# skypilot-org/skypilot

Hardware: AMD Instinct MI355X
Metric: tokens/sec (node) sky-launched Llama-3-8B (higher is better)
Workload: dtype bf16; 1 GPU; model=llama3-8b, global_batch=6, seq_len=4096, parallelism=dp1, sky_launched=True

## Files before the change

### skypilot_amd/models/llama.py

```python
from __future__ import annotations

import math
from dataclasses import dataclass

import torch
import torch.nn as nn

from skypilot_amd import ops


@dataclass
class LlamaConfig:
    name: str = "llama3-8b"
    vocab_size: int = 128256
    hidden_size: int = 4096
    intermediate_size: int = 14336
    num_layers: int = 32
    num_heads: int = 32
    num_kv_heads: int = 8
    head_dim: int = 128
    rope_theta: float = 500000.0
    norm_eps: float = 1e-5
    max_seq_len: int = 8192
    tie_embeddings: bool = False
# ... 100 lines not shown
        k = lin(x, self.wk.weight, self.wk.bias).view(B, S, self.n_kv, d)
        v = lin(x, self.wv.weight, self.wv.bias).view(B, S, self.n_kv, d)
        q = ops.rope(q.reshape(B * S, self.n_q, d), cos, sin,
                     positions).view(B, S, self.n_q, d)
        k = ops.rope(k.reshape(B * S, self.n_kv, d), cos, sin,
                     positions).view(B, S, self.n_kv, d)
        if infer_ctx is None:
            o = ops.attention(q, k, v, self.scale, causal=True)
        elif infer_ctx.mode == "append":
            o = append_attention(self, q, k, v, infer_ctx)
        else:
            slots = (infer_ctx.prefill_slots
                     if infer_ctx.prefill_slots is not None
                     else [infer_ctx.prefill_slot])
            lens = (infer_ctx.prefill_lens
                    if infer_ctx.prefill_lens is not None
                    else [infer_ctx.prefill_len])
            for i, (slot, ln) in enumerate(zip(slots, lens)):
                infer_ctx.cache.write_prefill(self.layer_idx, slot,
                                              k[i:i + 1], v[i:i + 1], ln)
            o = ops.attention(q, k, v, self.scale, causal=True)
        return lin(o.reshape(B, S, self.n_q * d), self.wo.weight)


class MLP(nn.Module):
    def __init__(self, cfg: LlamaConfig):
        super().__init__()
        h, m = cfg.hidden_size, cfg.intermediate_size
        self.w_gate_up = nn.Linear(h, 2 * m, bias=False)
        self.w_down = nn.Linear(m, h, bias=False)
        self.m = m

    def forward(self, x, infer_ctx=None):
        decode = infer_ctx is not None and infer_ctx.mode == "decode"
        lin = ops.decode_linear if decode else torch.nn.functional.linear
        return lin(ops.swiglu(lin(x, self.w_gate_up.weight)),
                   self.w_down.weight)

    def down_from_gu(self, gu):
        return ops.decode_linear(ops.swiglu(gu), self.w_down.weight)



class Block(nn.Module):
    def __init__(self, cfg: LlamaConfig, layer_idx: int):
        super().__init__()
        self.attn = Attention(cfg)
        self.attn.layer_idx = layer_idx
        self.mlp = MLP(cfg)
        self.attn_norm = nn.Parameter(torch.ones(cfg.hidden_size))
        self.mlp_norm = nn.Parameter(torch.ones(cfg.hidden_size))
        self.eps = cfg.norm_eps

    def forward(self, x, cos, sin, positions, infer_ctx=None):
        x = x + self.attn(ops.rmsnorm(x, self.attn_norm, self.eps), cos, sin,
                          positions, infer_ctx)
        x = x + self.mlp(ops.rmsnorm(x, self.mlp_norm, self.eps),
                         infer_ctx)
        return x


class Llama(nn.Module):
    def __init__(self, cfg: LlamaConfig):
        super().__init__()
        self.cfg = cfg
        self.embed = nn.Embedding(cfg.vocab_size, cfg.hidden_size)
        self.blocks = nn.ModuleList(
            Block(cfg, i) for i in range(cfg.num_layers))
        self.final_norm = nn.Parameter(torch.ones(cfg.hidden_size))
        self.lm_head = nn.Linear(cfg.hidden_size, cfg.vocab_size, bias=False)
        if cfg.tie_embeddings:
            self.lm_head.weight = self.embed.weight
        self._rope = None

    def _tables(self, device):
        if self._rope is None or self._rope[0].device != device:
            self._rope = rope_tables(self.cfg, device)
        return self._rope

    def forward(self, tokens: torch.Tensor, positions: torch.Tensor = None,
                infer_ctx=None) -> torch.Tensor:
        B, S = tokens.shape
        cos, sin = self._tables(tokens.device)
        if positions is None:
            positions = torch.arange(S, dtype=torch.int32,
                                     device=tokens.device)
            positions = positions.unsqueeze(0).expand(B, S).reshape(-1)
        x = self.embed(tokens)
        if infer_ctx is not None and infer_ctx.mode == "decode":
            res = None
            for blk in self.blocks:
                if not hasattr(blk.attn, "_wqkv"):
                    if res is None:
                        h = ops.rmsnorm(x, blk.attn_norm, blk.eps)
                    else:
                        x, h = ops.rmsnorm_res(x, res, blk.attn_norm,
                                               blk.eps)
                    a = blk.attn(h, cos, sin, positions, infer_ctx)
                    x, h2 = ops.rmsnorm_res(x, a, blk.mlp_norm, blk.eps)
                    res = blk.mlp(h2, infer_ctx)
                    continue
                x, qkv = ops.decode_norm_linear(
                    x, res, blk.attn_norm, blk.eps, blk.attn.packed_qkv())
                a = blk.attn(None, cos, sin, positions, infer_ctx,
                             qkv=qkv)
                x, gu = ops.decode_norm_linear(
                    x, a, blk.mlp_norm, blk.eps, blk.mlp.w_gate_up.weight)
                res = blk.mlp.down_from_gu(gu)
            _, logits = ops.decode_norm_linear(
                x, res, self.final_norm, self.cfg.norm_eps,
                self.lm_head.weight)
            return logits
        for blk in self.blocks:
            x = blk(x, cos, sin, positions, infer_ctx)
        if infer_ctx is not None and infer_ctx.mode == "append":
            last = (infer_ctx.append_lens.long() - 1).clamp(min=0)
            x = x[torch.arange(B, device=x.device), last].unsqueeze(1)
        x = ops.rmsnorm(x, self.final_norm, self.cfg.norm_eps)
        return self.lm_head(x)

    def loss(self, tokens: torch.Tensor, targets: torch.Tensor):
        logits = self.forward(tokens)
        return ops.fused_cross_entropy(
            logits.reshape(-1, self.cfg.vocab_size), targets.reshape(-1))

    def num_params(self) -> int:
        return sum(p.numel() for p in self.parameters())

    def flops_per_token(self, seq_len: int) -> float:
        c = self.cfg
        return 6 * self.num_params() + \
            6 * c.num_layers * 2 * seq_len * c.num_heads * c.head_dim


def build_model(name: str, device="cpu", dtype=torch.bfloat16,
                seed: int = 0) -> Llama:
    cfg = CONFIGS[name]
    torch.manual_seed(seed)
    with torch.device("meta" if device != "cpu" else "cpu"):
        model = Llama(cfg)
    if device != "cpu":
        model = model.to_empty(device=device)
        with torch.no_grad():
            for p in model.parameters():
                p.normal_(0.0, 0.02)
    return model.to(dtype)
```

### skypilot_amd/ops/__init__.py

```python
from __future__ import annotations

import importlib.util
import math
import os
from pathlib import Path

import torch

_C = None
_LOAD_ERR: Exception | None = None


def _load():
    global _C, _LOAD_ERR
    if _C is not None:
        return _C
    so = Path(__file__).resolve().parent / "_C.so"
    try:
        if not so.exists():
            raise ImportError(
                f"native extension {so} not built; run "
                "`python -m skypilot_amd.ops.build`")
        spec = importlib.util.spec_from_file_location("skypilot_amd.ops._C",
                                                      so)
# ... 57 lines not shown
    att = torch.matmul(qf, kf.transpose(-1, -2)) * scale
    if causal:
        mask = torch.triu(torch.ones(S, S, dtype=torch.bool,
                                     device=q.device), 1)
        att = att.masked_fill(mask, float("-inf"))
    p = att.softmax(-1)
    out = torch.matmul(p, vf)
    return out.permute(0, 2, 1, 3).to(q.dtype)


def cross_entropy_ref(logits: torch.Tensor, targets: torch.Tensor,
                      ignore_index: int = -100) -> torch.Tensor:
    return torch.nn.functional.cross_entropy(
        logits.float(), targets.long(), ignore_index=ignore_index,
        reduction="mean")


class _RMSNormFn(torch.autograd.Function):
    @staticmethod
    def forward(ctx, x, w, eps):
        if x.is_cuda:
            C = _require_native("rmsnorm")
            inv_rms = torch.empty(x.numel() // x.shape[-1],
                                  device=x.device, dtype=torch.float32)
            y = C.rmsnorm_fwd(x.contiguous(), w.contiguous(), inv_rms, eps)
            ctx.save_for_backward(x, w, inv_rms)
            ctx.native = True
            return y
        ctx.save_for_backward(x, w)
        ctx.eps = eps
        ctx.native = False
        return rmsnorm_ref(x, w, eps)

    @staticmethod
    def backward(ctx, dy):
        if ctx.native:
            x, w, inv_rms = ctx.saved_tensors
            C = native()
            dx, dw = C.rmsnorm_bwd(x.contiguous(), w.contiguous(),
                                   dy.contiguous(), inv_rms)
            return dx, dw.to(w.dtype), None
        x, w = ctx.saved_tensors
        xf, wf, dyf = x.float(), w.float(), dy.float()
        H = x.shape[-1]
        inv = torch.rsqrt(xf.pow(2).mean(-1, keepdim=True) + ctx.eps)
        dot = (dyf * wf * xf).sum(-1, keepdim=True)
        dx = inv * (dyf * wf - xf * inv * inv * dot / H)
        dw = (dyf * xf * inv).reshape(-1, H).sum(0)
        return dx.to(x.dtype), dw.to(w.dtype), None


def rmsnorm(x: torch.Tensor, w: torch.Tensor, eps: float = 1e-5):
    return _RMSNormFn.apply(x, w, eps)


class _RoPEFn(torch.autograd.Function):
    @staticmethod
    def forward(ctx, x, cos, sin, positions):
        ctx.save_for_backward(cos, sin, positions)
        if x.is_cuda:
            C = _require_native("rope")
            return C.rope(x.contiguous(), cos, sin, positions, False)
        return rope_ref(x, cos, sin, positions)

    @staticmethod
    def backward(ctx, dy):
        cos, sin, positions = ctx.saved_tensors
        if dy.is_cuda:
            C = native()
            return C.rope(dy.contiguous(), cos, sin, positions,
                          True), None, None, None
        return rope_ref(dy, cos, sin, positions, backward=True), \
            None, None, None


def rope(x, cos, sin, positions):
    if x.is_cuda and x.dim() > 3:
        positions = positions.expand(x.shape[:-2]).reshape(-1)
    return _RoPEFn.apply(x, cos, sin, positions)


class _AttentionFn(torch.autograd.Function):
    @staticmethod
    def forward(ctx, q, k, v, scale, causal):
        ctx.scale, ctx.causal = scale, causal
        if q.is_cuda:
            C = _require_native("attention")
            q, k, v = q.contiguous(), k.contiguous(), v.contiguous()
            O, lse = C.attn_fwd(q, k, v, scale, causal)
            ctx.save_for_backward(q, k, v, O, lse)
            ctx.native = True
            return O
        ctx.save_for_backward(q, k, v)
        ctx.native = False
        return attention_ref(q, k, v, scale, causal)

    @staticmethod
    def backward(ctx, dO):
        if ctx.native:
            q, k, v, O, lse = ctx.saved_tensors
            C = native()
            dq, dk, dv = C.attn_bwd(q, k, v, O, dO.contiguous(), lse,
                                    ctx.scale, ctx.causal)
            return dq, dk, dv, None, None
        q, k, v = ctx.saved_tensors
        with torch.enable_grad():
# ... 354 lines not shown

def sample_tokens(logits, temperature, top_p, top_k, seed, counter):
    if not logits.is_cuda:
        return sample_tokens_reference(logits, temperature, top_p, top_k,
                                       seed, counter)
    C = _require_native("sample_tokens")
    if logits.dtype != torch.bfloat16 or logits.dim() != 2:
        raise ValueError("sample_tokens: logits must be bf16 [n, V] on GPU")
    n = logits.shape[0]
    blk = pack_samp(n, temperature, top_p, top_k, seed,
                    counter).to(logits.device)
    toks, tau = C.sample_tokens(logits.contiguous(), blk[:5], blk[5])
    return toks, tau


def decode_sample_advance(logits, stage, ring, ctr, samp):
    C = _require_native("decode_sample_advance")
    C.decode_sample_advance(logits.contiguous(), stage, ring, ctr, samp)


def decode_swiglu_down(gu, weight):
    return decode_linear(swiglu(gu), weight)


def attn_decode_qkv(qkv, kc, vc, cos, sin, positions, kv_lens, slot_ids,
                    Hq, Hkv, scale):
    D = kc.shape[3]
    if qkv.is_cuda and qkv.dtype == torch.bfloat16 and D == 128:
        C = _require_native("attn_decode_qkv")
        return C.attn_decode_qkv(qkv.contiguous(), kc, vc, cos, sin,
                                 positions.int(), kv_lens.int(),
                                 slot_ids.int(), Hq, Hkv, scale)
    q = rope_kvwrite(qkv, kc, vc, cos, sin, positions, slot_ids, Hq, Hkv)
    return attn_decode(q, kc, vc, kv_lens, slot_ids, scale)


def rope_kvwrite(qkv, kc, vc, cos, sin, positions, slot_ids, Hq, Hkv):
    D = kc.shape[3]
    n = qkv.shape[0]
    if qkv.is_cuda and qkv.dtype == torch.bfloat16 and D == 128:
        C = _require_native("rope_kvwrite")
        return C.rope_kvwrite(qkv.contiguous(), kc, vc, cos, sin,
                              positions.int(), slot_ids.int(), Hq, Hkv)
    q, k, v = qkv.split([Hq * D, Hkv * D, Hkv * D], dim=-1)
    qr = rope(q.reshape(n, Hq, D), cos, sin, positions)
    kr = rope(k.reshape(n, Hkv, D), cos, sin, positions)
    pos = positions.long()
    kc[slot_ids.long(), pos] = kr
    vc[slot_ids.long(), pos] = v.reshape(n, Hkv, D)
    return qr


__all__ = [
    "rmsnorm", "rope", "attention", "fused_cross_entropy", "attn_decode",
    "swiglu", "decode_linear", "rmsnorm_res", "rope_kvwrite",
    "decode_swiglu_down",
    "native", "native_available", "rmsnorm_ref", "rope_ref",
    "attention_ref", "cross_entropy_ref", "attn_decode_ref",
    "attn_append", "attn_append_ref",
]
```

### skypilot_amd/ops/csrc/bindings.cpp

```cpp
#include <torch/extension.h>

#include <ATen/hip/HIPContext.h>
#include <hip/hip_runtime.h>

#include <limits>
#include <vector>

#include "attn_append.h"
#include "attn_launch.h"

#define CHECK_GPU(x) TORCH_CHECK(x.is_cuda(), #x " must be on GPU")
#define CHECK_CONTIG(x) TORCH_CHECK(x.is_contiguous(), #x " must be contiguous")
#define CHECK_BF16(x) \
  TORCH_CHECK(x.scalar_type() == at::kBFloat16, #x " must be bf16")

static hipStream_t cur_stream() {
  return at::hip::getCurrentHIPStream().stream();
}

extern "C" {
void rmsnorm_fwd_launch(const void*, const void*, void*, float*, long long,
                        int, float, hipStream_t);
void rmsnorm_bwd_launch(const void*, const void*, const void*, const float*,
                        void*, float*, long long, int, hipStream_t);
void rope_launch(const void*, void*, const float*, const float*, const int*,
                 long long, int, int, bool, hipStream_t);
void adamw_launch(void*, float*, const void*, float*, float*, long long,
                  float, float, float, float, float, int, float, hipStream_t);
void cross_entropy_launch(void*, const int*, float*, long long, int, float,
                          int, hipStream_t);
void mfma_probe_launch(const void*, const void*, float*, hipStream_t);
void mfma32_probe_launch(const void*, const void*, float*, hipStream_t);
void trb16_probe_launch(float*, int, hipStream_t);
void permlane_probe_launch(float*, hipStream_t);
void skinny_gemm_launch(const void*, const void*, void*, int, int, int,
                        hipStream_t);
void skinny_gemm_swiglu_launch(const void*, const void*, void*, int, int,
                               int, hipStream_t);
void transpose_bf16_launch(const void*, void*, int, int, hipStream_t);
void skinny_gemm_fp8_launch(const void*, const float*, const void*, void*,
                            int, int, int, hipStream_t);
void gemm_nt_launch(const void*, const void*, void*, int, int, long long,
                    hipStream_t);
void adamw_mt_launch(const void*, const void*, const void*, const void*,
                     const void*, long long, float, float, float, float,
                     int, float, hipStream_t);
void decode_advance_launch(const void*, long long, void*, long long,
                           void*, const void*, int, hipStream_t);
void sample_tokens_launch(const void*, int, long long, const void*,
                          const void*, void*, void*, hipStream_t);
void decode_sample_advance_launch(const void*, int, void*, long long, void*,
                                  const void*, int, const void*,
                                  hipStream_t);
void rmsnorm_res_launch(const void*, const void*, const void*, void*, void*,
                        int, int, float, hipStream_t);
void rope_kvwrite_launch(const void*, void*, void*, void*, const void*,
                         const void*, const void*, const void*, int, int,
                         int, int, int, hipStream_t);
void swiglu_fwd_launch(const void*, void*, long long, int, hipStream_t);
void swiglu_bwd_launch(const void*, const void*, void*, long long, int,
                       hipStream_t);
void skinny_gemm_fp8_norm_launch(const void*, const float*, const void*,
                                 const void*, const void*, void*, float,
                                 void*, int, int, int, hipStream_t);
void attn_decode_qkv_launch(const void*, void*, void*, void*, const void*,
                            const void*, const int*, const int*,
                            const int*, int, int, int, int, float,
                            hipStream_t);
void attn_decode_launch(const void*, const void*, const void*, void*,
                        const int*, const int*, int, int, int, int, float,
                        hipStream_t);
}

torch::Tensor rmsnorm_fwd(torch::Tensor x, torch::Tensor w,
                          torch::Tensor inv_rms, double eps) {
  CHECK_GPU(x); CHECK_CONTIG(x); CHECK_BF16(x);
  CHECK_GPU(w); CHECK_CONTIG(w); CHECK_BF16(w);
  const int H = (int)x.size(-1);
  TORCH_CHECK(H % 8 == 0, "hidden dim must be a multiple of 8");
  TORCH_CHECK(w.numel() == H, "rmsnorm_fwd: w must have H = ", H,
              " elements, got ", w.numel());
  long long rows = x.numel() / H;
  CHECK_GPU(inv_rms); CHECK_CONTIG(inv_rms);
  TORCH_CHECK(inv_rms.scalar_type() == at::kFloat && inv_rms.numel() == rows,
              "rmsnorm_fwd: inv_rms must be fp32 with one entry per row");
  auto y = torch::empty_like(x);
  rmsnorm_fwd_launch(x.data_ptr(), w.data_ptr(), y.data_ptr(),
                     inv_rms.data_ptr<float>(), rows, H, (float)eps,
                     cur_stream());
  return y;
}

std::vector<torch::Tensor> rmsnorm_bwd(torch::Tensor x, torch::Tensor w,
                                       torch::Tensor dy,
                                       torch::Tensor inv_rms) {
  CHECK_GPU(x); CHECK_CONTIG(x); CHECK_BF16(x);
  CHECK_GPU(w); CHECK_CONTIG(w); CHECK_BF16(w);
  CHECK_GPU(dy); CHECK_CONTIG(dy); CHECK_BF16(dy);
  CHECK_GPU(inv_rms); CHECK_CONTIG(inv_rms);
  const int H = (int)x.size(-1);
  TORCH_CHECK(H % 8 == 0 && H <= 16384,
              "rmsnorm_bwd: hidden dim must be a multiple of 8 and at most "
              "16384, got ", H);
  TORCH_CHECK(w.numel() == H, "rmsnorm_bwd: w must have H = ", H,
              " elements, got ", w.numel());
  TORCH_CHECK(dy.sizes() == x.sizes(), "rmsnorm_bwd: dy must have x's shape");
  long long rows = x.numel() / H;
  TORCH_CHECK(inv_rms.scalar_type() == at::kFloat && inv_rms.numel() == rows,
              "rmsnorm_bwd: inv_rms must be fp32 with one entry per row");
  auto dx = torch::empty_like(x);
  auto dw = torch::zeros({(long)H},
                         x.options().dtype(at::kFloat));
  rmsnorm_bwd_launch(x.data_ptr(), w.data_ptr(), dy.data_ptr(),
                     inv_rms.data_ptr<float>(), dx.data_ptr(),
                     dw.data_ptr<float>(), rows, H, cur_stream());
  return {dx, dw};
}

torch::Tensor rope(torch::Tensor x, torch::Tensor cos_tab,
                   torch::Tensor sin_tab, torch::Tensor positions,
                   bool backward) {
  CHECK_GPU(x); CHECK_CONTIG(x); CHECK_BF16(x);
  TORCH_CHECK(positions.scalar_type() == at::kInt,
              "rope: positions must be int32");
  CHECK_GPU(positions); CHECK_CONTIG(positions);
  TORCH_CHECK(x.dim() >= 2, "rope: x must be [..., heads, head_dim]");
  const int D = (int)x.size(-1);
  const int H = (int)x.size(-2);
  TORCH_CHECK(D % 2 == 0, "rope: head dim must be even, got ", D);
  long long n_tokens = x.numel() / ((long long)H * D);
  TORCH_CHECK(positions.numel() == n_tokens, "rope: need one position per "
              "token: ", n_tokens, " tokens, ", positions.numel(),
              " positions");
  for (const torch::Tensor& t : {cos_tab, sin_tab}) {
    CHECK_GPU(t); CHECK_CONTIG(t);
    TORCH_CHECK(t.scalar_type() == at::kFloat, "rope: cos/sin must be fp32");
    TORCH_CHECK(t.dim() >= 1 && t.size(-1) == D / 2,
                "rope: cos/sin last dim must be head_dim/2 = ", D / 2);
  }
  auto y = torch::empty_like(x);
  rope_launch(x.data_ptr(), y.data_ptr(), cos_tab.data_ptr<float>(),
              sin_tab.data_ptr<float>(), positions.data_ptr<int>(), n_tokens,
              H, D, backward, cur_stream());
  return y;
}

void adamw_step(std::vector<torch::Tensor> params_bf16,
                std::vector<torch::Tensor> params_master,
                std::vector<torch::Tensor> grads,
                std::vector<torch::Tensor> exp_avg,
                std::vector<torch::Tensor> exp_avg_sq, double lr, double beta1,
                double beta2, double eps, double weight_decay, int64_t step,
                double grad_scale, std::vector<bool> decay_mask) {
  auto stream = cur_stream();
  for (size_t i = 0; i < params_bf16.size(); ++i) {
    auto& p = params_bf16[i];
    long long n = p.numel();
    float wd = decay_mask.empty() || decay_mask[i] ? (float)weight_decay : 0.f;
    adamw_launch(p.data_ptr(), params_master[i].data_ptr<float>(),
                 grads[i].data_ptr(), exp_avg[i].data_ptr<float>(),
                 exp_avg_sq[i].data_ptr<float>(), n, (float)lr, (float)beta1,
                 (float)beta2, (float)eps, wd, (int)step, (float)grad_scale,
                 stream);
  }
}

torch::Tensor cross_entropy_fused(torch::Tensor logits, torch::Tensor targets,
                                  double grad_scale, int64_t ignore_index) {
  CHECK_GPU(logits); CHECK_CONTIG(logits); CHECK_BF16(logits);
// ... 397 lines not shown
  const int64_t N = X.size(0), I = X.size(1);
  TORCH_CHECK(N >= 1 && N <= 8, op, ": N must be 1..8, got ", N);
  TORCH_CHECK(I >= 16 && I % 16 == 0 &&
                  I <= std::numeric_limits<int>::max(),
              op, ": I must be a positive multiple of 16, got ", I);
  check_fp8_weight(op, W8, scale, I, X);
  const int64_t O = W8.size(0);
  auto y = torch::empty({N, O}, X.options());
  skinny_gemm_fp8_launch(W8.data_ptr(), scale.data_ptr<float>(),
                         X.data_ptr(), y.data_ptr(), (int)N, (int)I, (int)O,
                         cur_stream());
  return y;
}

torch::Tensor skinny_gemm(torch::Tensor X, torch::Tensor W) {
  CHECK_GPU(X); CHECK_CONTIG(X); CHECK_BF16(X);
  CHECK_GPU(W); CHECK_CONTIG(W); CHECK_BF16(W);
  const int N = (int)X.size(0), I = (int)X.size(1), O = (int)W.size(0);
  TORCH_CHECK(W.size(1) == I, "skinny_gemm: inner dims mismatch");
  TORCH_CHECK(N >= 1 && N <= 8, "skinny_gemm: N must be 1..8");
  TORCH_CHECK(I % 512 == 0, "skinny_gemm: I must be a multiple of 512");
  auto y = torch::empty({N, O}, X.options());
  skinny_gemm_launch(W.data_ptr(), X.data_ptr(), y.data_ptr(), N, I, O,
                     cur_stream());
  return y;
}

std::vector<torch::Tensor> rmsnorm_res(torch::Tensor x, torch::Tensor res,
                                       torch::Tensor w, double eps) {
  const char* op = "rmsnorm_res";
  check_dense(op, "x", x, at::kBFloat16, x);
  TORCH_CHECK(x.dim() >= 1, op, ": x must be [..., H], got a scalar");
  const int64_t H = x.size(-1);
  TORCH_CHECK(H >= 256 && H % 256 == 0 && H <= 8192, op,
              ": H must be a multiple of 256 and <= 8192, got ", H);
  check_dense(op, "res", res, at::kBFloat16, x);
  TORCH_CHECK(res.sizes() == x.sizes(), op, ": res must have x's shape ",
              x.sizes(), ", got ", res.sizes());
  check_dense(op, "w", w, at::kBFloat16, x);
  TORCH_CHECK(w.numel() == H, op, ": w must have H = ", H,
              " elements, got ", w.numel());
  const int64_t rows = x.numel() / H;
  TORCH_CHECK(rows <= std::numeric_limits<int>::max(), op, ": ", rows,
              " rows exceed the grid limit 2^31 - 1");
  auto x_out = torch::empty_like(x);
  auto h_out = torch::empty_like(x);
  if (rows > 0)
    rmsnorm_res_launch(x.data_ptr(), res.data_ptr(), w.data_ptr(),
                       x_out.data_ptr(), h_out.data_ptr(), (int)rows, (int)H,
                       (float)eps, cur_stream());
  return {x_out, h_out};
}

void decode_advance(torch::Tensor logits, torch::Tensor stage,
                    torch::Tensor ring, torch::Tensor ctr) {
  const char* op = "decode_advance";
  check_dense(op, "logits", logits, at::kBFloat16, logits);
  TORCH_CHECK(logits.dim() >= 1, op,
              ": logits must be [b, V], got a scalar");
  const int64_t V = logits.size(-1);
  TORCH_CHECK(V >= 1 && V <= std::numeric_limits<int>::max(), op,
              ": V must be in [1, 2^31 - 1], got ", V);
  const int64_t b = logits.numel() / V;
  check_dense(op, "stage", stage, at::kInt, logits);
  TORCH_CHECK(stage.dim() == 2 && stage.size(0) == 6 && stage.size(1) == b,
              op, ": stage must be [6, b] = [6, ", b, "], got ",
              stage.sizes());
  check_dense(op, "ring", ring, at::kLong, logits);
  TORCH_CHECK(ring.dim() == 2 && ring.size(0) >= 1 &&
                  ring.size(0) <= std::numeric_limits<int>::max() &&
                  ring.size(1) == b,
              op, ": ring must be [chunk >= 1, b] = [chunk, ", b, "], got ",
              ring.sizes());
  check_dense(op, "ctr", ctr, at::kLong, logits);
  TORCH_CHECK(ctr.numel() == 1, op, ": ctr must hold one element, got ",
              ctr.sizes());
  TORCH_CHECK(b <= std::numeric_limits<int>::max(), op, ": b = ", b,
              " rows exceed the grid limit 2^31 - 1");
  if (b > 0)
    decode_advance_launch(logits.data_ptr(), V, stage.data_ptr(), b,
                          ring.data_ptr(), ctr.data_ptr(),
                          (int)ring.size(0), cur_stream());
}

static const long long kSampleMaxV = 1ll << 23;

std::vector<torch::Tensor> sample_tokens(torch::Tensor logits,
                                         torch::Tensor samp,
                                         torch::Tensor counter) {
  CHECK_GPU(logits); CHECK_CONTIG(logits); CHECK_BF16(logits);
  CHECK_GPU(samp); CHECK_CONTIG(samp);
  CHECK_GPU(counter); CHECK_CONTIG(counter);
  TORCH_CHECK(logits.dim() == 2, "sample_tokens: logits must be [n, V]");
  TORCH_CHECK(samp.dtype() == torch::kInt32, "sample_tokens: samp int32");
  TORCH_CHECK(counter.dtype() == torch::kInt32,
              "sample_tokens: counter int32");
  const long long n = logits.size(0);
  const long long V = logits.size(1);
  TORCH_CHECK(V >= 1 && V <= kSampleMaxV,
              "sample_tokens: V must be in [1, 2^23], got ", V);
  TORCH_CHECK(samp.dim() == 2 && samp.size(0) == 5 && samp.size(1) == n,
              "sample_tokens: samp must be [5, n]");
  TORCH_CHECK(counter.dim() == 1 && counter.size(0) == n,
              "sample_tokens: counter must be [n]");
  auto tokens = torch::empty({n}, logits.options().dtype(torch::kInt64));
  auto tau = torch::empty({n}, logits.options().dtype(torch::kFloat));
// ... 79 lines not shown

torch::Tensor swiglu_bwd(torch::Tensor gu, torch::Tensor dy) {
  CHECK_GPU(gu); CHECK_CONTIG(gu); CHECK_BF16(gu);
  CHECK_GPU(dy); CHECK_CONTIG(dy); CHECK_BF16(dy);
  const int M2 = (int)gu.size(-1);
  TORCH_CHECK(M2 % 16 == 0, "swiglu_bwd: last dim must be 2*M with "
              "M % 8 == 0, got ", M2);
  auto ysizes = gu.sizes().vec();
  ysizes.back() = M2 / 2;
  TORCH_CHECK(dy.sizes() == at::IntArrayRef(ysizes),
              "swiglu_bwd: dy must have the shape of swiglu_fwd(gu)");
  long long rows = gu.numel() / M2;
  auto dgu = torch::empty_like(gu);
  swiglu_bwd_launch(gu.data_ptr(), dy.data_ptr(), dgu.data_ptr(), rows,
                    M2 / 2, cur_stream());
  return dgu;
}

torch::Tensor mfma_probe(torch::Tensor A, torch::Tensor B) {
  CHECK_GPU(A); CHECK_BF16(A); CHECK_CONTIG(A); CHECK_CONTIG(B);
  TORCH_CHECK(A.size(0) == 16 && A.size(1) == 32);
  TORCH_CHECK(B.size(0) == 32 && B.size(1) == 16);
  auto C = torch::zeros({16, 16}, A.options().dtype(at::kFloat));
  mfma_probe_launch(A.data_ptr(), B.data_ptr(), C.data_ptr<float>(),
                    cur_stream());
  return C;
}

torch::Tensor mfma32_probe(torch::Tensor A, torch::Tensor B) {
  CHECK_GPU(A); CHECK_BF16(A); CHECK_CONTIG(A); CHECK_CONTIG(B);
  TORCH_CHECK(A.size(0) == 32 && A.size(1) == 16);
  TORCH_CHECK(B.size(0) == 16 && B.size(1) == 32);
  auto C = torch::zeros({32, 32}, A.options().dtype(at::kFloat));
  mfma32_probe_launch(A.data_ptr(), B.data_ptr(), C.data_ptr<float>(),
                      cur_stream());
  return C;
}

torch::Tensor trb16_probe(int64_t mode, torch::Tensor ref_dev) {
  auto out = torch::zeros({64, 4}, ref_dev.options().dtype(at::kFloat));
  trb16_probe_launch(out.data_ptr<float>(), (int)mode, cur_stream());
  return out;
}

torch::Tensor permlane_probe(torch::Tensor ref_dev) {
  auto out = torch::zeros({64, 2}, ref_dev.options().dtype(at::kFloat));
  permlane_probe_launch(out.data_ptr<float>(), cur_stream());
  return out;
}

PYBIND11_MODULE(TORCH_EXTENSION_NAME, m) {
  m.def("rmsnorm_fwd", &rmsnorm_fwd);
  m.def("rmsnorm_bwd", &rmsnorm_bwd);
  m.def("rope", &rope);
  m.def("adamw_step", &adamw_step);
  m.def("cross_entropy_fused", &cross_entropy_fused);
  m.def("attn_fwd", &attn_fwd);
  m.def("attn_bwd", &attn_bwd, py::arg("Q"), py::arg("K"), py::arg("V"),
        py::arg("O"), py::arg("dO"), py::arg("lse"), py::arg("scale"),
        py::arg("causal"), py::arg("dkv_variant") = -1,
        py::arg("dq_variant") = -1);
  m.def("attn_decode", &attn_decode);
  m.def("attn_append", &attn_append);
  m.def("skinny_gemm", &skinny_gemm);
  m.def("skinny_gemm_fp8", &skinny_gemm_fp8);
  m.def("transpose_bf16", &transpose_bf16);
  m.def("gemm_nt", &gemm_nt);
  m.def("wgrad_tn", &wgrad_tn);
  m.def("adamw_step_mt", &adamw_step_mt);
  m.def("skinny_gemm_swiglu", &skinny_gemm_swiglu);
  m.def("rmsnorm_res", &rmsnorm_res);
  m.def("rope_kvwrite", &rope_kvwrite);
  m.def("decode_advance", &decode_advance);
  m.def("sample_tokens", &sample_tokens);
  m.def("decode_sample_advance", &decode_sample_advance);
  m.def("attn_decode_qkv", &attn_decode_qkv);
  m.def("skinny_gemm_fp8_norm", &skinny_gemm_fp8_norm);
  m.def("swiglu_fwd", &swiglu_fwd);
  m.def("swiglu_bwd", &swiglu_bwd);
  m.def("mfma_probe", &mfma_probe);
  m.def("mfma32_probe", &mfma32_probe);
  m.def("trb16_probe", &trb16_probe);
  m.def("permlane_probe", &permlane_probe);
}
```

### skypilot_amd/ops/csrc/rmsnorm.hip

```cpp
#include "common.h"

extern "C" __global__ void rmsnorm_fwd_kernel(
    const unsigned short* __restrict__ x, const unsigned short* __restrict__ w,
    unsigned short* __restrict__ y, float* __restrict__ inv_rms, int rows,
    int H, float eps) {
  __shared__ float red[16];
  const int nvec = H / 8;
  for (int row = blockIdx.x; row < rows; row += gridDim.x) {
    const s16x8* xrow = (const s16x8*)(x + (long long)row * H);
    s16x8* yrow = (s16x8*)(y + (long long)row * H);
    float ss = 0.f;
    for (int v = threadIdx.x; v < nvec; v += blockDim.x) {
      s16x8 xv = xrow[v];
      float f[8];
      bf8_to_f32(xv, f);
#pragma unroll
      for (int i = 0; i < 8; ++i) ss += f[i] * f[i];
    }
    ss = block_reduce_sum(ss, red);
    float inv = rsqrtf(ss / (float)H + eps);
    if (threadIdx.x == 0 && inv_rms) inv_rms[row] = inv;
    for (int v = threadIdx.x; v < nvec; v += blockDim.x) {
      s16x8 xv = xrow[v];
      s16x8 wv = ((const s16x8*)w)[v];
      float f[8];
#pragma unroll
      for (int i = 0; i < 8; ++i)
        f[i] = bf2f((unsigned short)xv[i]) * inv * bf2f((unsigned short)wv[i]);
      yrow[v] = f32_to_bf8(f);
    }
    __syncthreads();
  }
}

template <int NV>
__global__ void rmsnorm_bwd_kernel(
    const unsigned short* __restrict__ x, const unsigned short* __restrict__ w,
    const unsigned short* __restrict__ dy, const float* __restrict__ inv_rms,
    unsigned short* __restrict__ dx, float* __restrict__ dw, int rows, int H) {
  __shared__ float red[16];
  const int nvec = H / 8;
  float dw_acc[NV][8];
#pragma unroll
  for (int v = 0; v < NV; ++v)
#pragma unroll
    for (int i = 0; i < 8; ++i) dw_acc[v][i] = 0.f;

  for (int row = blockIdx.x; row < rows; row += gridDim.x) {
    const s16x8* xrow = (const s16x8*)(x + (long long)row * H);
    const s16x8* dyrow = (const s16x8*)(dy + (long long)row * H);
    s16x8* dxrow = (s16x8*)(dx + (long long)row * H);
    const float inv = inv_rms[row];

    float xf[NV][8], dyf[NV][8], wf[NV][8];
    float dot = 0.f;
#pragma unroll
    for (int v = 0; v < NV; ++v) {
      int idx = threadIdx.x + v * blockDim.x;
      if (idx < nvec) {
        bf8_to_f32(xrow[idx], xf[v]);
        bf8_to_f32(dyrow[idx], dyf[v]);
        bf8_to_f32(((const s16x8*)w)[idx], wf[v]);
#pragma unroll
        for (int i = 0; i < 8; ++i) dot += dyf[v][i] * wf[v][i] * xf[v][i];
      }
    }
    dot = block_reduce_sum(dot, red);
    const float k = dot * inv * inv / (float)H;
#pragma unroll
    for (int v = 0; v < NV; ++v) {
      int idx = threadIdx.x + v * blockDim.x;
      if (idx < nvec) {
        float out[8];
#pragma unroll
        for (int i = 0; i < 8; ++i) {
          out[i] = inv * (dyf[v][i] * wf[v][i] - xf[v][i] * k);
          dw_acc[v][i] += dyf[v][i] * xf[v][i] * inv;
        }
        dxrow[idx] = f32_to_bf8(out);
      }
    }
    __syncthreads();
  }
#pragma unroll
  for (int v = 0; v < NV; ++v) {
    int idx = threadIdx.x + v * blockDim.x;
    if (idx < nvec) {
#pragma unroll
      for (int i = 0; i < 8; ++i) atomicAdd(&dw[idx * 8 + i], dw_acc[v][i]);
    }
  }
}

extern "C" void rmsnorm_fwd_launch(const void* x, const void* w, void* y,
                                   float* inv_rms, long long rows, int H,
                                   float eps, hipStream_t stream) {
  int grid = rows < 2048 ? (int)rows : 2048;
  hipLaunchKernelGGL(rmsnorm_fwd_kernel, dim3(grid), dim3(256), 0, stream,
                     (const unsigned short*)x, (const unsigned short*)w,
                     (unsigned short*)y, inv_rms, (int)rows, H, eps);
}

extern "C" void rmsnorm_bwd_launch(const void* x, const void* w,
                                   const void* dy, const float* inv_rms,
                                   void* dx, float* dw, long long rows, int H,
                                   hipStream_t stream) {
  int grid = rows < 512 ? (int)rows : 512;
  const int nvec = H / 8;
  dim3 b(256);
#define LAUNCH(NV)                                                          \
  hipLaunchKernelGGL((rmsnorm_bwd_kernel<NV>), dim3(grid), b, 0, stream,    \
                     (const unsigned short*)x, (const unsigned short*)w,    \
                     (const unsigned short*)dy, inv_rms,                    \
                     (unsigned short*)dx, dw, (int)rows, H)
  if (nvec <= 256) LAUNCH(1);
  else if (nvec <= 512) LAUNCH(2);
  else if (nvec <= 1024) LAUNCH(4);
  else LAUNCH(8);
#undef LAUNCH
}
```

Baseline: 21160 tokens/s.

## Fuse residual add into RMSNorm and restructure RMSNorm backward with per-wave rows

The training forward now defers each block's residual add and fuses it into the next RMSNorm through a new add_rmsnorm op, which has a native forward kernel and a backward that folds the residual gradient into dx. The RMSNorm backward kernel is rewritten so each wavefront handles one row when H<=4096, using a wave reduction instead of a block reduction with syncthreads. Per-block dw partials are written to a buffer and summed by a separate reduce kernel, replacing per-element atomicAdds. This cuts elementwise add kernels and memory traffic, at the cost of an extra partial buffer, a second launch in backward, and a bf16 rounding point on dx+g that differs slightly from before.

```diff
diff --git a/skypilot_amd/models/llama.py b/skypilot_amd/models/llama.py
--- a/skypilot_amd/models/llama.py
+++ b/skypilot_amd/models/llama.py
@@ -176,12 +176,18 @@
         self.mlp_norm = nn.Parameter(torch.ones(cfg.hidden_size))
         self.eps = cfg.norm_eps
 
+    def forward_res(self, x, res, cos, sin, positions, infer_ctx=None):
+        if res is None:
+            h = ops.rmsnorm(x, self.attn_norm, self.eps)
+        else:
+            x, h = ops.add_rmsnorm(x, res, self.attn_norm, self.eps)
+        a = self.attn(h, cos, sin, positions, infer_ctx)
+        x, h = ops.add_rmsnorm(x, a, self.mlp_norm, self.eps)
+        return x, self.mlp(h, infer_ctx)
+
     def forward(self, x, cos, sin, positions, infer_ctx=None):
-        x = x + self.attn(ops.rmsnorm(x, self.attn_norm, self.eps), cos, sin,
-                          positions, infer_ctx)
-        x = x + self.mlp(ops.rmsnorm(x, self.mlp_norm, self.eps),
-                         infer_ctx)
-        return x
+        x, pending = self.forward_res(x, None, cos, sin, positions, infer_ctx)
+        return x + pending
 
 
 class Llama(nn.Module):
@@ -235,12 +241,25 @@
                 x, res, self.final_norm, self.cfg.norm_eps,
                 self.lm_head.weight)
             return logits
+        res = None
         for blk in self.blocks:
-            x = blk(x, cos, sin, positions, infer_ctx)
+            if hasattr(blk, "forward_res"):
+                x, res = blk.forward_res(x, res, cos, sin, positions,
+                                         infer_ctx)
+            else:
+                if res is not None:
+                    x, res = x + res, None
+                x = blk(x, cos, sin, positions, infer_ctx)
         if infer_ctx is not None and infer_ctx.mode == "append":
+            if res is not None:
+                x, res = x + res, None
             last = (infer_ctx.append_lens.long() - 1).clamp(min=0)
             x = x[torch.arange(B, device=x.device), last].unsqueeze(1)
-        x = ops.rmsnorm(x, self.final_norm, self.cfg.norm_eps)
+        if res is None:
+            x = ops.rmsnorm(x, self.final_norm, self.cfg.norm_eps)
+        else:
+            _, x = ops.add_rmsnorm(x, res, self.final_norm,
+                                   self.cfg.norm_eps)
         return self.lm_head(x)
 
     def loss(self, tokens: torch.Tensor, targets: torch.Tensor):
diff --git a/skypilot_amd/ops/__init__.py b/skypilot_amd/ops/__init__.py
--- a/skypilot_amd/ops/__init__.py
+++ b/skypilot_amd/ops/__init__.py
@@ -133,6 +133,44 @@
 
 def rmsnorm(x: torch.Tensor, w: torch.Tensor, eps: float = 1e-5):
     return _RMSNormFn.apply(x, w, eps)
+
+
+class _AddRMSNormFn(torch.autograd.Function):
+
+    @staticmethod
+    def forward(ctx, x, res, w, eps):
+        C = _require_native("add_rmsnorm")
+        inv_rms = torch.empty(x.numel() // x.shape[-1],
+                              device=x.device, dtype=torch.float32)
+        x2, h = C.rmsnorm_res_fwd(x.contiguous(), res.contiguous(),
+                                  w.contiguous(), inv_rms, eps)
+        ctx.save_for_backward(x2, w, inv_rms)
+        ctx.set_materialize_grads(False)
+        return x2, h
+
+    @staticmethod
+    def backward(ctx, g_x2, g_h):
+        x2, w, inv_rms = ctx.saved_tensors
+        if g_h is None:
+            if g_x2 is None:
+                return None, None, None, None
+            return g_x2, g_x2, torch.zeros_like(w), None
+        C = native()
+        if g_x2 is None:
+            dx, dw = C.rmsnorm_bwd(x2, w.contiguous(), g_h.contiguous(),
+                                   inv_rms)
+        else:
+            dx, dw = C.rmsnorm_bwd_res(x2, w.contiguous(), g_h.contiguous(),
+                                       inv_rms, g_x2.contiguous())
+        return dx, dx, dw.to(w.dtype), None
+
+
+def add_rmsnorm(x: torch.Tensor, res: torch.Tensor, w: torch.Tensor,
+                eps: float = 1e-5):
+    if x.is_cuda:
+        return _AddRMSNormFn.apply(x, res, w, eps)
+    x2 = x + res
+    return x2, rmsnorm(x2, w, eps)
 
 
 class _RoPEFn(torch.autograd.Function):
@@ -593,7 +631,7 @@
 
 
 __all__ = [
-    "rmsnorm", "rope", "attention", "fused_cross_entropy", "attn_decode",
+    "rmsnorm", "add_rmsnorm", "rope", "attention", "fused_cross_entropy", "attn_decode",
     "swiglu", "decode_linear", "rmsnorm_res", "rope_kvwrite",
     "decode_swiglu_down",
     "native", "native_available", "rmsnorm_ref", "rope_ref",
diff --git a/skypilot_amd/ops/csrc/bindings.cpp b/skypilot_amd/ops/csrc/bindings.cpp
--- a/skypilot_amd/ops/csrc/bindings.cpp
+++ b/skypilot_amd/ops/csrc/bindings.cpp
@@ -21,8 +21,13 @@
 extern "C" {
 void rmsnorm_fwd_launch(const void*, const void*, void*, float*, long long,
                         int, float, hipStream_t);
+void rmsnorm_res_fwd_launch(const void*, const void*, const void*, void*,
+                            void*, float*, long long, int, float,
+                            hipStream_t);
+int rmsnorm_bwd_grid(long long, int);
 void rmsnorm_bwd_launch(const void*, const void*, const void*, const float*,
-                        void*, float*, long long, int, hipStream_t);
+                        const void*, void*, float*, float*, long long, int,
+                        hipStream_t);
 void rope_launch(const void*, void*, const float*, const float*, const int*,
                  long long, int, int, bool, hipStream_t);
 void adamw_launch(void*, float*, const void*, float*, float*, long long,
@@ -91,6 +96,22 @@
   return y;
 }
 
+static std::vector<torch::Tensor> rmsnorm_bwd_run(
+    const torch::Tensor& x, const torch::Tensor& w, const torch::Tensor& dy,
+    const torch::Tensor& inv_rms, const torch::Tensor* g, int H,
+    long long rows) {
+  auto dx = torch::empty_like(x);
+  auto dw = torch::empty({(long)H}, x.options().dtype(at::kFloat));
+  if (rows == 0) return {dx, dw.zero_()};
+  auto part = torch::empty({(long)rmsnorm_bwd_grid(rows, H), (long)H},
+                           dw.options());
+  rmsnorm_bwd_launch(x.data_ptr(), w.data_ptr(), dy.data_ptr(),
+                     inv_rms.data_ptr<float>(), g ? g->data_ptr() : nullptr,
+                     dx.data_ptr(), part.data_ptr<float>(),
+                     dw.data_ptr<float>(), rows, H, cur_stream());
+  return {dx, dw};
+}
+
 std::vector<torch::Tensor> rmsnorm_bwd(torch::Tensor x, torch::Tensor w,
                                        torch::Tensor dy,
                                        torch::Tensor inv_rms) {
@@ -108,13 +129,7 @@
   long long rows = x.numel() / H;
   TORCH_CHECK(inv_rms.scalar_type() == at::kFloat && inv_rms.numel() == rows,
               "rmsnorm_bwd: inv_rms must be fp32 with one entry per row");
-  auto dx = torch::empty_like(x);
-  auto dw = torch::zeros({(long)H},
-                         x.options().dtype(at::kFloat));
-  rmsnorm_bwd_launch(x.data_ptr(), w.data_ptr(), dy.data_ptr(),
-                     inv_rms.data_ptr<float>(), dx.data_ptr(),
-                     dw.data_ptr<float>(), rows, H, cur_stream());
-  return {dx, dw};
+  return rmsnorm_bwd_run(x, w, dy, inv_rms, nullptr, H, rows);
 }
 
 torch::Tensor rope(torch::Tensor x, torch::Tensor cos_tab,
@@ -618,6 +633,70 @@
   return {x_out, h_out};
 }
 
+static int64_t check_norm_x(const char* op, const torch::Tensor& x,
+                            int64_t max_H) {
+  check_dense(op, "x", x, at::kBFloat16, x);
+  TORCH_CHECK(x.dim() >= 1, op, ": x must be [..., H], got a scalar");
+  const int64_t H = x.size(-1);
+  TORCH_CHECK(H >= 8 && H % 8 == 0 && H <= max_H, op,
+              ": H must be a multiple of 8 and at most ", max_H, ", got ", H);
+  return H;
+}
+
+static void check_norm_args(const char* op, const torch::Tensor& x,
+                            const torch::Tensor& w,
+                            const torch::Tensor& inv_rms, int64_t H) {
+  check_dense(op, "w", w, at::kBFloat16, x);
+  TORCH_CHECK(w.numel() == H, op, ": w must have H = ", H,
+              " elements, got ", w.numel());
+  check_dense(op, "inv_rms", inv_rms, at::kFloat, x);
+  TORCH_CHECK(inv_rms.numel() == x.numel() / H, op,
+              ": inv_rms must have one entry per row (", x.numel() / H,
+              "), got ", inv_rms.numel());
+}
+
+std::vector<torch::Tensor> rmsnorm_res_fwd(torch::Tensor x, torch::Tensor res,
+                                           torch::Tensor w,
+                                           torch::Tensor inv_rms, double eps) {
+  const char* op = "rmsnorm_res_fwd";
+  const int64_t H =
+      check_norm_x(op, x, std::numeric_limits<int>::max() / 8 * 8);
+  check_dense(op, "res", res, at::kBFloat16, x);
+  TORCH_CHECK(res.sizes() == x.sizes(), op, ": res must have x's shape ",
+              x.sizes(), ", got ", res.sizes());
+  check_norm_args(op, x, w, inv_rms, H);
+  const int64_t rows = x.numel() / H;
+  TORCH_CHECK(rows <= std::numeric_limits<int>::max(), op, ": ", rows,
+              " rows exceed the kernel's limit 2^31 - 1");
+  auto x2 = torch::empty_like(x);
+  auto h = torch::empty_like(x);
+  if (rows > 0)
+    rmsnorm_res_fwd_launch(x.data_ptr(), res.data_ptr(), w.data_ptr(),
+                           x2.data_ptr(), h.data_ptr(),
+                           inv_rms.data_ptr<float>(), rows, (int)H, (float)eps,
+                           cur_stream());
+  return {x2, h};
+}
+
+std::vector<torch::Tensor> rmsnorm_bwd_res(torch::Tensor x, torch::Tensor w,
+                                           torch::Tensor dy,
+                                           torch::Tensor inv_rms,
+                                           torch::Tensor g) {
+  const char* op = "rmsnorm_bwd_res";
+  const int64_t H = check_norm_x(op, x, 16384);
+  check_norm_args(op, x, w, inv_rms, H);
+  check_dense(op, "dy", dy, at::kBFloat16, x);
+  TORCH_CHECK(dy.sizes() == x.sizes(), op, ": dy must have x's shape ",
+              x.sizes(), ", got ", dy.sizes());
+  check_dense(op, "g", g, at::kBFloat16, x);
+  TORCH_CHECK(g.sizes() == x.sizes(), op, ": g must have x's shape ",
+              x.sizes(), ", got ", g.sizes());
+  const int64_t rows = x.numel() / H;
+  TORCH_CHECK(rows <= std::numeric_limits<int>::max(), op, ": ", rows,
+              " rows exceed the kernel's limit 2^31 - 1");
+  return rmsnorm_bwd_run(x, w, dy, inv_rms, &g, (int)H, rows);
+}
+
 void decode_advance(torch::Tensor logits, torch::Tensor stage,
                     torch::Tensor ring, torch::Tensor ctr) {
   const char* op = "decode_advance";
@@ -803,6 +882,8 @@
 PYBIND11_MODULE(TORCH_EXTENSION_NAME, m) {
   m.def("rmsnorm_fwd", &rmsnorm_fwd);
   m.def("rmsnorm_bwd", &rmsnorm_bwd);
+  m.def("rmsnorm_res_fwd", &rmsnorm_res_fwd);
+  m.def("rmsnorm_bwd_res", &rmsnorm_bwd_res);
   m.def("rope", &rope);
   m.def("adamw_step", &adamw_step);
   m.def("cross_entropy_fused", &cross_entropy_fused);
diff --git a/skypilot_amd/ops/csrc/rmsnorm.hip b/skypilot_amd/ops/csrc/rmsnorm.hip
--- a/skypilot_amd/ops/csrc/rmsnorm.hip
+++ b/skypilot_amd/ops/csrc/rmsnorm.hip
@@ -1,7 +1,9 @@
 #include "common.h"
 
-extern "C" __global__ void rmsnorm_fwd_kernel(
-    const unsigned short* __restrict__ x, const unsigned short* __restrict__ w,
+template <bool HAS_RES>
+__device__ __forceinline__ void rmsnorm_fwd_body(
+    const unsigned short* __restrict__ x, const unsigned short* __restrict__ res,
+    const unsigned short* __restrict__ w, unsigned short* x2,
     unsigned short* __restrict__ y, float* __restrict__ inv_rms, int rows,
     int H, float eps) {
   __shared__ float red[16];
@@ -14,14 +16,25 @@
       s16x8 xv = xrow[v];
       float f[8];
       bf8_to_f32(xv, f);
+      if (HAS_RES) {
+        float r[8];
+        bf8_to_f32(((const s16x8*)(res + (long long)row * H))[v], r);
+#pragma unroll
+        for (int i = 0; i < 8; ++i) f[i] += r[i];
+        xv = f32_to_bf8(f);
+        ((s16x8*)(x2 + (long long)row * H))[v] = xv;
+        bf8_to_f32(xv, f);
+      }
 #pragma unroll
       for (int i = 0; i < 8; ++i) ss += f[i] * f[i];
     }
     ss = block_reduce_sum(ss, red);
     float inv = rsqrtf(ss / (float)H + eps);
     if (threadIdx.x == 0 && inv_rms) inv_rms[row] = inv;
+    const s16x8* nrow =
+        HAS_RES ? (const s16x8*)(x2 + (long long)row * H) : xrow;
     for (int v = threadIdx.x; v < nvec; v += blockDim.x) {
-      s16x8 xv = xrow[v];
+      s16x8 xv = nrow[v];
       s16x8 wv = ((const s16x8*)w)[v];
       float f[8];
 #pragma unroll
@@ -33,62 +46,194 @@
   }
 }
 
-template <int NV>
-__global__ void rmsnorm_bwd_kernel(
+extern "C" __global__ void rmsnorm_fwd_kernel(
+    const unsigned short* __restrict__ x, const unsigned short* __restrict__ w,
+    unsigned short* __restrict__ y, float* __restrict__ inv_rms, int rows,
+    int H, float eps) {
+  rmsnorm_fwd_body<false>(x, nullptr, w, nullptr, y, inv_rms, rows, H, eps);
+}
+
+extern "C" __global__ void rmsnorm_res_fwd_kernel(
+    const unsigned short* __restrict__ x, const unsigned short* __restrict__ res,
+    const unsigned short* __restrict__ w, unsigned short* x2,
+    unsigned short* __restrict__ y, float* __restrict__ inv_rms, int rows,
+    int H, float eps) {
+  rmsnorm_fwd_body<true>(x, res, w, x2, y, inv_rms, rows, H, eps);
+}
+
+#define RMS_BWD_THREADS 256
+
+template <int NV, int GS, bool HAS_RES>
+__device__ __forceinline__ void rmsnorm_bwd_body(
     const unsigned short* __restrict__ x, const unsigned short* __restrict__ w,
     const unsigned short* __restrict__ dy, const float* __restrict__ inv_rms,
-    unsigned short* __restrict__ dx, float* __restrict__ dw, int rows, int H) {
-  __shared__ float red[16];
+    const unsigned short* __restrict__ g, unsigned short* __restrict__ dx,
+    float* __restrict__ dw_part, int rows, int H) {
+  constexpr int GROUPS = RMS_BWD_THREADS / GS;
+  extern __shared__ __attribute__((aligned(16))) float smem[];
   const int nvec = H / 8;
+  const int lane = threadIdx.x % GS;
+  const int group = threadIdx.x / GS;
+
   float dw_acc[NV][8];
-#pragma unroll
-  for (int v = 0; v < NV; ++v)
+  s16x8 wv[NV];
+#pragma unroll
+  for (int v = 0; v < NV; ++v) {
+    const int idx = lane + v * GS;
 #pragma unroll
     for (int i = 0; i < 8; ++i) dw_acc[v][i] = 0.f;
-
-  for (int row = blockIdx.x; row < rows; row += gridDim.x) {
-    const s16x8* xrow = (const s16x8*)(x + (long long)row * H);
-    const s16x8* dyrow = (const s16x8*)(dy + (long long)row * H);
-    s16x8* dxrow = (s16x8*)(dx + (long long)row * H);
+    wv[v] = idx < nvec ? ((const s16x8*)w)[idx] : (s16x8)(0);
+  }
+
+  for (long long row = (long long)blockIdx.x * GROUPS + group; row < rows;
+       row += (long long)gridDim.x * GROUPS) {
+    const s16x8* xrow = (const s16x8*)(x + row * H);
+    const s16x8* dyrow = (const s16x8*)(dy + row * H);
+    const s16x8* grow = HAS_RES ? (const s16x8*)(g + row * H) : nullptr;
+    s16x8* dxrow = (s16x8*)(dx + row * H);
+
+    s16x8 xv[NV], dyv[NV], gv[NV];
+#pragma unroll
+    for (int v = 0; v < NV; ++v) {
+      const int idx = lane + v * GS;
+      xv[v] = dyv[v] = gv[v] = (s16x8)(0);
+      if (idx < nvec) {
+        xv[v] = xrow[idx];
+        dyv[v] = dyrow[idx];
+        if (HAS_RES) gv[v] = grow[idx];
+      }
+    }
     const float inv = inv_rms[row];
-
-    float xf[NV][8], dyf[NV][8], wf[NV][8];
     float dot = 0.f;
 #pragma unroll
     for (int v = 0; v < NV; ++v) {
-      int idx = threadIdx.x + v * blockDim.x;
+      if (lane + v * GS < nvec) {
+#pragma unroll
+        for (int i = 0; i < 8; ++i)
+          dot += bf2f((unsigned short)dyv[v][i]) *
+                 bf2f((unsigned short)wv[v][i]) *
+                 bf2f((unsigned short)xv[v][i]);
+      }
+    }
+    if (GS == WAVE) dot = wave_reduce_sum(dot);
+    else dot = block_reduce_sum(dot, smem);
+    const float k = dot * inv * inv / (float)H;
+#pragma unroll
+    for (int v = 0; v < NV; ++v)
+      asm volatile("" : "+v"(xv[v]), "+v"(dyv[v]), "+v"(wv[v]));
+#pragma unroll
+    for (int v = 0; v < NV; ++v) {
+      const int idx = lane + v * GS;
       if (idx < nvec) {
-        bf8_to_f32(xrow[idx], xf[v]);
-        bf8_to_f32(dyrow[idx], dyf[v]);
-        bf8_to_f32(((const s16x8*)w)[idx], wf[v]);
-#pragma unroll
-        for (int i = 0; i < 8; ++i) dot += dyf[v][i] * wf[v][i] * xf[v][i];
-      }
-    }
-    dot = block_reduce_sum(dot, red);
-    const float k = dot * inv * inv / (float)H;
+        s16x8 ov;
+#pragma unroll
+        for (int i = 0; i < 8; ++i) {
+          const float xf = bf2f((unsigned short)xv[v][i]);
+          const float dyf = bf2f((unsigned short)dyv[v][i]);
+          const float wf = bf2f((unsigned short)wv[v][i]);
+          unsigned short o = f2bf(inv * (dyf * wf - xf * k));
+          if (HAS_RES) o = f2bf(bf2f(o) + bf2f((unsigned short)gv[v][i]));
+          ov[i] = (short)o;
+          dw_acc[v][i] += dyf * xf * inv;
+        }
+        dxrow[idx] = ov;
+      }
+    }
+  }
+
+  float* out = dw_part + (long long)blockIdx.x * H;
+  if (GROUPS == 1) {
 #pragma unroll
     for (int v = 0; v < NV; ++v) {
-      int idx = threadIdx.x + v * blockDim.x;
+      const int idx = lane + v * GS;
       if (idx < nvec) {
-        float out[8];
-#pragma unroll
-        for (int i = 0; i < 8; ++i) {
-          out[i] = inv * (dyf[v][i] * wf[v][i] - xf[v][i] * k);
-          dw_acc[v][i] += dyf[v][i] * xf[v][i] * inv;
+        f32x4* o = (f32x4*)(out + idx * 8);
+        o[0] = f32x4{dw_acc[v][0], dw_acc[v][1], dw_acc[v][2], dw_acc[v][3]};
+        o[1] = f32x4{dw_acc[v][4], dw_acc[v][5], dw_acc[v][6], dw_acc[v][7]};
+      }
+    }
+  } else {
+    for (int gi = 0; gi < GROUPS; ++gi) {
+      if (group == gi) {
+#pragma unroll
+        for (int v = 0; v < NV; ++v) {
+          const int idx = lane + v * GS;
+          if (idx < nvec) {
+            f32x4* s = (f32x4*)(smem + idx * 8);
+            f32x4 a = f32x4{dw_acc[v][0], dw_acc[v][1], dw_acc[v][2],
+                            dw_acc[v][3]};
+            f32x4 b = f32x4{dw_acc[v][4], dw_acc[v][5], dw_acc[v][6],
+                            dw_acc[v][7]};
+            if (gi > 0) {
+              a += s[0];
+              b += s[1];
+            }
+            s[0] = a;
+            s[1] = b;
+          }
         }
-        dxrow[idx] = f32_to_bf8(out);
-      }
-    }
-    __syncthreads();
-  }
-#pragma unroll
-  for (int v = 0; v < NV; ++v) {
-    int idx = threadIdx.x + v * blockDim.x;
-    if (idx < nvec) {
-#pragma unroll
-      for (int i = 0; i < 8; ++i) atomicAdd(&dw[idx * 8 + i], dw_acc[v][i]);
-    }
+      }
+      __syncthreads();
+    }
+    for (int c = threadIdx.x; c < H / 4; c += RMS_BWD_THREADS)
+      ((f32x4*)out)[c] = ((const f32x4*)smem)[c];
+  }
+}
+
+#define RMS_BWD_KERNEL(NAME, NV, GS)                                          \
+  extern "C" __global__ void __launch_bounds__(RMS_BWD_THREADS, 2)            \
+  rmsnorm_bwd_##NAME(const unsigned short* __restrict__ x,                    \
+                     const unsigned short* __restrict__ w,                    \
+                     const unsigned short* __restrict__ dy,                   \
+                     const float* __restrict__ inv_rms,                       \
+                     unsigned short* __restrict__ dx,                         \
+                     float* __restrict__ dw_part, int rows, int H) {          \
+    rmsnorm_bwd_body<NV, GS, false>(x, w, dy, inv_rms, nullptr, dx, dw_part,  \
+                                    rows, H);                                 \
+  }                                                                           \
+  extern "C" __global__ void __launch_bounds__(RMS_BWD_THREADS, 2)            \
+  rmsnorm_bwd_res_##NAME(const unsigned short* __restrict__ x,                \
+                         const unsigned short* __restrict__ w,                \
+                         const unsigned short* __restrict__ dy,               \
+                         const float* __restrict__ inv_rms,                   \
+                         const unsigned short* __restrict__ g,                \
+                         unsigned short* __restrict__ dx,                     \
+                         float* __restrict__ dw_part, int rows, int H) {      \
+    rmsnorm_bwd_body<NV, GS, true>(x, w, dy, inv_rms, g, dx, dw_part, rows,   \
+                                   H);                                        \
+  }
+
+RMS_BWD_KERNEL(wave_nv1, 1, 64)
+RMS_BWD_KERNEL(wave_nv2, 2, 64)
+RMS_BWD_KERNEL(wave_nv4, 4, 64)
+RMS_BWD_KERNEL(wave_nv8, 8, 64)
+RMS_BWD_KERNEL(block_nv4, 4, 256)
+RMS_BWD_KERNEL(block_nv8, 8, 256)
+#undef RMS_BWD_KERNEL
+
+#define RMS_RED_WAVES 16
+
+extern "C" __global__ void __launch_bounds__(RMS_RED_WAVES * WAVE)
+rmsnorm_dw_reduce_kernel(const float* __restrict__ part,
+                         float* __restrict__ dw, int nparts, int H) {
+  __shared__ f32x4 fold[RMS_RED_WAVES][WAVE];
+  const int lane = threadIdx.x & (WAVE - 1);
+  const int wid = threadIdx.x / WAVE;
+  const int col = blockIdx.x * WAVE + lane;
+  const int ncol = H / 4;
+  f32x4 acc = {0.f, 0.f, 0.f, 0.f};
+  if (col < ncol) {
+#pragma unroll 4
+    for (int r = wid; r < nparts; r += RMS_RED_WAVES)
+      acc += ((const f32x4*)(part + (long long)r * H))[col];
+  }
+  fold[wid][lane] = acc;
+  __syncthreads();
+  if (wid == 0 && col < ncol) {
+    f32x4 s = fold[0][lane];
+#pragma unroll
+    for (int j = 1; j < RMS_RED_WAVES; ++j) s += fold[j][lane];
+    ((f32x4*)dw)[col] = s;
   }
 }
 
@@ -101,21 +246,56 @@
                      (unsigned short*)y, inv_rms, (int)rows, H, eps);
 }
 
+extern "C" void rmsnorm_res_fwd_launch(const void* x, const void* res,
+                                       const void* w, void* x2, void* y,
+                                       float* inv_rms, long long rows, int H,
+                                       float eps, hipStream_t stream) {
+  int grid = rows < 2048 ? (int)rows : 2048;
+  hipLaunchKernelGGL(rmsnorm_res_fwd_kernel, dim3(grid), dim3(256), 0, stream,
+                     (const unsigned short*)x, (const unsigned short*)res,
+                     (const unsigned short*)w, (unsigned short*)x2,
+                     (unsigned short*)y, inv_rms, (int)rows, H, eps);
+}
+
+extern "C" int rmsnorm_bwd_grid(long long rows, int H) {
+  const long long per_block = H <= 4096 ? RMS_BWD_THREADS / WAVE : 1;
+  long long grid = (rows + per_block - 1) / per_block;
+  return grid < 512 ? (int)grid : 512;
+}
+
 extern "C" void rmsnorm_bwd_launch(const void* x, const void* w,
                                    const void* dy, const float* inv_rms,
-                                   void* dx, float* dw, long long rows, int H,
+                                   const void* g, void* dx, float* dw_part,
+                                   float* dw, long long rows, int H,
                                    hipStream_t stream) {
-  int grid = rows < 512 ? (int)rows : 512;
+  const int grid = rmsnorm_bwd_grid(rows, H);
   const int nvec = H / 8;
-  dim3 b(256);
-#define LAUNCH(NV)                                                          \
-  hipLaunchKernelGGL((rmsnorm_bwd_kernel<NV>), dim3(grid), b, 0, stream,    \
-                     (const unsigned short*)x, (const unsigned short*)w,    \
-                     (const unsigned short*)dy, inv_rms,                    \
-                     (unsigned short*)dx, dw, (int)rows, H)
-  if (nvec <= 256) LAUNCH(1);
-  else if (nvec <= 512) LAUNCH(2);
-  else if (nvec <= 1024) LAUNCH(4);
-  else LAUNCH(8);
+  const bool wave_row = H <= 4096;
+  const size_t lds = wave_row ? (size_t)H * sizeof(float) : 16 * sizeof(float);
+  dim3 b(RMS_BWD_THREADS);
+#define LAUNCH(NAME)                                                        \
+  do {                                                                      \
+    if (g)                                                                  \
+      hipLaunchKernelGGL(rmsnorm_bwd_res_##NAME, dim3(grid), b, lds, stream, \
+                         (const unsigned short*)x, (const unsigned short*)w, \
+                         (const unsigned short*)dy, inv_rms,                \
+                         (const unsigned short*)g, (unsigned short*)dx,     \
+                         dw_part, (int)rows, H);                            \
+    else                                                                    \
+      hipLaunchKernelGGL(rmsnorm_bwd_##NAME, dim3(grid), b, lds, stream,    \
+                         (const unsigned short*)x, (const unsigned short*)w, \
+                         (const unsigned short*)dy, inv_rms,                \
+                         (unsigned short*)dx, dw_part, (int)rows, H);       \
+  } while (0)
+  if (nvec <= 64) LAUNCH(wave_nv1);
+  else if (nvec <= 128) LAUNCH(wave_nv2);
+  else if (nvec <= 256) LAUNCH(wave_nv4);
+  else if (nvec <= 512) LAUNCH(wave_nv8);
+  else if (nvec <= 1024) LAUNCH(block_nv4);
+  else LAUNCH(block_nv8);
 #undef LAUNCH
-}
+  const int ncol = H / 4;
+  hipLaunchKernelGGL(rmsnorm_dw_reduce_kernel, dim3((ncol + WAVE - 1) / WAVE),
+                     dim3(RMS_RED_WAVES * WAVE), 0, stream,
+                     (const float*)dw_part, dw, grid, H);
+}
```

Measured after the change: 21290 tokens/s (median of 6 runs). Within noise of the previous version (+0.6%).
